# microsoft/GenerativeImage2Text

Hardware: AMD Instinct MI355X
Metric: captions/sec whole-node (GIT_BASE 224px bs=64/GPU greedy len=20) (higher is better)
Workload: dtype f16; 1 GPU; GIT_BASE 224px bs=64/GPU greedy max_len=20 frames=1; global_batch=64, parallelism=dp1, decode_steps_per_caption=19, seq_len_returned=20, hip_graph=True, contexts_in_flight=4, layernorm_folded=True, library=libgitmi_f16.so, encoder_chains=2, schedule=mixed

## Files before the change

generativeimage2text_amd/csrc/kernels_attn.hip:

```cpp
#include "gitmi_common.h"
#include "launchers.h"
#include <type_traits>

namespace gitmi {

constexpr int HD = 64;

template <typename T>
__global__ __launch_bounds__(256) void attn_full_valu_kernel(AttnFullArgs a) {
    __shared__ float Ks[64][HD + 1];
    __shared__ float Vs[64][HD + 1];
    __shared__ float qs[16][HD];
    __shared__ float ps[16][64];

    const int tid = threadIdx.x, lane = tid & 63, wave = tid >> 6;
    const int h = blockIdx.y, b = blockIdx.z;
    const int q0 = blockIdx.x * 16;
    const T* Q = reinterpret_cast<const T*>(a.q);
    const T* K = reinterpret_cast<const T*>(a.k);
    const T* V = reinterpret_cast<const T*>(a.v);
    T* O = reinterpret_cast<T*>(a.out);
    const size_t base_row = (size_t)b * a.N;
    const int n = a.ntok ? a.ntok[b] : a.N;
    if (q0 >= n) {
        for (int i = tid; i < 16 * HD; i += 256) {
            const int qr = q0 + i / HD;
            if (qr < a.N) st<T>(O + (base_row + qr) * a.ldo + h * HD + i % HD, 0.f);
        }
        return;
    }

    for (int i = tid; i < 16 * HD; i += 256) {
        const int qi = i / HD, d = i % HD;
        const int qr = q0 + qi;
        qs[qi][d] = qr < n ? ld<T>(Q + (base_row + qr) * a.ldq + h * HD + d) * a.scale : 0.f;
    }

    float m_run[4], l_run[4], o_acc[4];
#pragma unroll
    for (int j = 0; j < 4; ++j) { m_run[j] = -INFINITY; l_run[j] = 0.f; o_acc[j] = 0.f; }

    for (int kt = 0; kt < n; kt += 64) {
        __syncthreads();
        for (int i = tid; i < 64 * HD; i += 256) {
            const int key = i / HD, d = i % HD;
            const int kr = kt + key;
            float kv = 0.f, vv = 0.f;
            if (kr < n) {
                kv = ld<T>(K + (base_row + kr) * a.ldk + h * HD + d);
                vv = ld<T>(V + (base_row + kr) * a.ldv + h * HD + d);
            }
            Ks[key][d] = kv;
            Vs[key][d] = vv;
        }
        __syncthreads();
#pragma unroll
        for (int j = 0; j < 4; ++j) {
            const int qi = wave * 4 + j;
            float s = 0.f;
#pragma unroll 16
            for (int d = 0; d < HD; ++d) s += qs[qi][d] * Ks[lane][d];
            if (kt + lane >= n) s = -INFINITY;
            const float m_new = fmaxf(m_run[j], wave_max(s));
            const float p = __expf(s - m_new);
            const float alpha = __expf(m_run[j] - m_new);
            l_run[j] = l_run[j] * alpha + wave_sum(p);
            m_run[j] = m_new;
            ps[qi][lane] = p;
            __builtin_amdgcn_fence(__ATOMIC_RELEASE, "wavefront");
            __builtin_amdgcn_wave_barrier();
            __builtin_amdgcn_fence(__ATOMIC_ACQUIRE, "wavefront");
            float o = o_acc[j] * alpha;
#pragma unroll 16
            for (int key = 0; key < 64; ++key) o += ps[qi][key] * Vs[key][lane];
            o_acc[j] = o;
        }
    }
#pragma unroll
    for (int j = 0; j < 4; ++j) {
        const int qr = q0 + wave * 4 + j;
        if (qr < a.N) st<T>(O + (base_row + qr) * a.ldo + h * HD + lane, qr < n ? o_acc[j] / l_run[j] : 0.f);
    }
}

constexpr int FA_LDK = HD + 8;
constexpr int FA_LDV = 64 + 8;

__global__ __launch_bounds__(256) void attn_full_mfma_kernel(AttnFullArgs a) {
    __shared__ __attribute__((aligned(16))) bf16_t Ks[64 * FA_LDK];
    __shared__ __attribute__((aligned(16))) bf16_t Vt[HD * FA_LDV];

    constexpr int QT = 4;
    const int tid = threadIdx.x, lane = tid & 63, wave = tid >> 6;
    const int l15 = lane & 15, lg = lane >> 4;
    const int h = blockIdx.y, b = blockIdx.z;
    const int qbase = blockIdx.x * 256;
    const bf16_t* Q = reinterpret_cast<const bf16_t*>(a.q);
    const bf16_t* K = reinterpret_cast<const bf16_t*>(a.k);
    const bf16_t* V = reinterpret_cast<const bf16_t*>(a.v);
    bf16_t* O = reinterpret_cast<bf16_t*>(a.out);
    const size_t base_row = (size_t)b * a.N;
    const int n = a.ntok ? a.ntok[b] : a.N;

    bf16x8_t qf[QT][2];
    f32x4_t o_acc[QT][4];
    float m_run[QT], l_run[QT];
#pragma unroll
    for (int t = 0; t < QT; ++t) {
        int qr = qbase + (t * 4 + wave) * 16 + l15;
        qr = qr < n ? qr : n - 1;
        const bf16_t* qp = Q + (base_row + qr) * a.ldq + h * HD + lg * 8;
        qf[t][0] = *reinterpret_cast<const bf16x8_t*>(qp);
        qf[t][1] = *reinterpret_cast<const bf16x8_t*>(qp + 32);
#pragma unroll
        for (int dt = 0; dt < 4; ++dt) o_acc[t][dt] = f32x4_t{0.f, 0.f, 0.f, 0.f};
        m_run[t] = -INFINITY;
        l_run[t] = 0.f;
    }

    const int ld_row = tid >> 3;
    const int ld_c = (tid & 7) * 8;

    const int kend = qbase < n ? n : 0;
    for (int kt = 0; kt < kend; kt += 64) {
        __syncthreads();
#pragma unroll
        for (int it = 0; it < 2; ++it) {
            const int key = ld_row + it * 32;
            int kr = kt + key;
            kr = kr < n ? kr : n - 1;
            const u32x4_t kc = *reinterpret_cast<const u32x4_t*>(K + (base_row + kr) * a.ldk + h * HD + ld_c);
            const u32x4_t vc = *reinterpret_cast<const u32x4_t*>(V + (base_row + kr) * a.ldv + h * HD + ld_c);
            *reinterpret_cast<u32x4_t*>(Ks + key * FA_LDK + ld_c) = kc;
#pragma unroll
            for (int e = 0; e < 4; ++e) {
                Vt[(ld_c + 2 * e) * FA_LDV + key] = (bf16_t)(vc[e] & 0xffffu);
                Vt[(ld_c + 2 * e + 1) * FA_LDV + key] = (bf16_t)(vc[e] >> 16);
            }
        }
        __syncthreads();

#pragma unroll
        for (int t = 0; t < QT; ++t) {
            if (qbase + (t * 4 + wave) * 16 >= n) continue;
            f32x4_t s_acc[4];
#pragma unroll
            for (int st_ = 0; st_ < 4; ++st_) {
                s_acc[st_] = f32x4_t{0.f, 0.f, 0.f, 0.f};
#pragma unroll
                for (int ks = 0; ks < 2; ++ks) {
                    const bf16x8_t kf = *reinterpret_cast<const bf16x8_t*>(Ks + (st_ * 16 + l15) * FA_LDK + ks * 32 + lg * 8);
                    s_acc[st_] = mfma16(kf, qf[t][ks], s_acc[st_]);
                }
            }
            float tmax = -INFINITY;
#pragma unroll
            for (int st_ = 0; st_ < 4; ++st_)
#pragma unroll
                for (int r = 0; r < 4; ++r) {
                    const int key = kt + st_ * 16 + lg * 4 + r;
                    const float sv = key < n ? s_acc[st_][r] * a.scale : -INFINITY;
                    s_acc[st_][r] = sv;
                    tmax = fmaxf(tmax, sv);
                }
            tmax = fmaxf(tmax, __shfl_xor(tmax, 16, 64));
            tmax = fmaxf(tmax, __shfl_xor(tmax, 32, 64));
            const float m_new = fmaxf(m_run[t], tmax);
            const float alpha = fast_exp(m_run[t] - m_new);
            float psum = 0.f;
#pragma unroll
            for (int st_ = 0; st_ < 4; ++st_)
#pragma unroll
                for (int r = 0; r < 4; ++r) {
                    const float p = fast_exp(s_acc[st_][r] - m_new);
                    s_acc[st_][r] = p;
                    psum += p;
                }
            psum += __shfl_xor(psum, 16, 64);
            psum += __shfl_xor(psum, 32, 64);
            l_run[t] = l_run[t] * alpha + psum;
            m_run[t] = m_new;
#pragma unroll
            for (int dt = 0; dt < 4; ++dt)
#pragma unroll
                for (int r = 0; r < 4; ++r) o_acc[t][dt][r] *= alpha;

#pragma unroll
            for (int hf = 0; hf < 2; ++hf) {
                bf16x8_t pf;
                {
                    union { bf16x8_t v; uint32_t u[4]; } pk;
                    pk.u[0] = pack2bf(s_acc[2 * hf][0], s_acc[2 * hf][1]);
                    pk.u[1] = pack2bf(s_acc[2 * hf][2], s_acc[2 * hf][3]);
                    pk.u[2] = pack2bf(s_acc[2 * hf + 1][0], s_acc[2 * hf + 1][1]);
                    pk.u[3] = pack2bf(s_acc[2 * hf + 1][2], s_acc[2 * hf + 1][3]);
                    pf = pk.v;
                }
#pragma unroll
                for (int dt = 0; dt < 4; ++dt) {
                    union { bf16x8_t v; uint2 h2[2]; } vf;
                    const bf16_t* vp = Vt + (dt * 16 + l15) * FA_LDV + hf * 32 + lg * 4;
                    vf.h2[0] = *reinterpret_cast<const uint2*>(vp);
                    vf.h2[1] = *reinterpret_cast<const uint2*>(vp + 16);
                    o_acc[t][dt] = mfma16(vf.v, pf, o_acc[t][dt]);
                }
            }
        }
    }

#pragma unroll
    for (int t = 0; t < QT; ++t) {
        const int qr = qbase + (t * 4 + wave) * 16 + l15;
        if (qr < a.N) {
            const float inv = qr < n ? 1.0f / l_run[t] : 0.f;
            bf16_t* op = O + (base_row + qr) * a.ldo + h * HD;
#pragma unroll
            for (int dt = 0; dt < 4; ++dt) {
                uint2 tt;
                tt.x = pack2bf(o_acc[t][dt][0] * inv, o_acc[t][dt][1] * inv);
                tt.y = pack2bf(o_acc[t][dt][2] * inv, o_acc[t][dt][3] * inv);
                *reinterpret_cast<uint2*>(op + dt * 16 + lg * 4) = tt;
            }
        }
    }
}

template <int NSUB, bool RAGGED = false>
__global__ __launch_bounds__(256, 2) void attn_full_mfma_short_kernel(AttnFullArgs a) {
    constexpr int NK = NSUB * 16;
    constexpr int NB = (NSUB + 1) / 2;
    constexpr int LDV = NB * 32 + 8;
    static_assert((LDV / 8) % 2 == 1, "V^T row stride must be an odd multiple of 16 bytes");
    __shared__ __attribute__((aligned(16))) bf16_t Ks[NK * FA_LDK];
    __shared__ __attribute__((aligned(16))) bf16_t Vt[HD * LDV];

    const int tid = threadIdx.x, lane = tid & 63, wave = tid >> 6;
    const int l15 = lane & 15, lg = lane >> 4;
    const int h = blockIdx.x, b = blockIdx.y;
    const bf16_t* Q = reinterpret_cast<const bf16_t*>(a.q);
    const bf16_t* K = reinterpret_cast<const bf16_t*>(a.k);
    const bf16_t* V = reinterpret_cast<const bf16_t*>(a.v);
    bf16_t* O = reinterpret_cast<bf16_t*>(a.out);
    const size_t base_row = (size_t)b * a.N;
    const int n = RAGGED ? a.ntok[b] : a.N;
    if constexpr (RAGGED) {
        for (int i = tid; i < (a.N - n) * 8; i += 256) {
            const int qr = n + (i >> 3);
            *reinterpret_cast<u32x4_t*>(O + (base_row + qr) * a.ldo + h * HD + (i & 7) * 8) = u32x4_t{0u, 0u, 0u, 0u};
        }
    }

#pragma unroll
    for (int it = 0; it < (NK * 8 + 255) / 256; ++it) {
        int idx = tid + it * 256;
        const bool ok = idx < NK * 8;
        idx = ok ? idx : NK * 8 - 1;
        const int key = idx >> 3, c = idx & 7;
        const int kr = key < n ? key : n - 1;
        const u32x4_t kc = *reinterpret_cast<const u32x4_t*>(K + (base_row + kr) * a.ldk + h * HD + c * 8);
        if (ok) *reinterpret_cast<u32x4_t*>(Ks + key * FA_LDK + c * 8) = kc;
    }
#pragma unroll
    for (int it = 0; it < (NB * 8 * 8 + 255) / 256; ++it) {
        int task = tid + it * 256;
        const bool ok = task < NB * 8 * 8;
        task = ok ? task : NB * 8 * 8 - 1;
        const int kg = task % (NB * 8), c = task / (NB * 8);
        u32x4_t vc[4];
#pragma unroll
        for (int e = 0; e < 4; ++e) {
            const int key = kg * 4 + e;
            const int kr = key < n ? key : n - 1;
            vc[e] = *reinterpret_cast<const u32x4_t*>(V + (base_row + kr) * a.ldv + h * HD + c * 8);
            if (key >= n) vc[e] = u32x4_t{0u, 0u, 0u, 0u};
        }
        if (ok) {
#pragma unroll
            for (int w = 0; w < 4; ++w) {
                uint2 even, odd;
                even.x = (vc[0][w] & 0xffffu) | (vc[1][w] << 16);
                even.y = (vc[2][w] & 0xffffu) | (vc[3][w] << 16);
                odd.x = (vc[0][w] >> 16) | (vc[1][w] & 0xffff0000u);
                odd.y = (vc[2][w] >> 16) | (vc[3][w] & 0xffff0000u);
                *reinterpret_cast<uint2*>(Vt + (c * 8 + 2 * w) * LDV + kg * 4) = even;
                *reinterpret_cast<uint2*>(Vt + (c * 8 + 2 * w + 1) * LDV + kg * 4) = odd;
            }
        }
    }
    __syncthreads();

    const int nqt = (n + 15) >> 4;
    const float c2 = a.scale * 1.4426950408889634f;

    auto process = [&](auto nt_c, int t0) {
        constexpr int NT = decltype(nt_c)::value;
        bf16x8_t qf[NT][2];
#pragma unroll
        for (int u = 0; u < NT; ++u) {
            int qr = (t0 + 4 * u) * 16 + l15;
            qr = qr < n ? qr : n - 1;
            const bf16_t* qp = Q + (base_row + qr) * a.ldq + h * HD + lg * 8;
            qf[u][0] = *reinterpret_cast<const bf16x8_t*>(qp);
            qf[u][1] = *reinterpret_cast<const bf16x8_t*>(qp + 32);
        }
        f32x4_t sacc[NT][NSUB];
#pragma unroll
        for (int st_ = 0; st_ < NSUB; ++st_) {
            const bf16x8_t kf0 = *reinterpret_cast<const bf16x8_t*>(Ks + (st_ * 16 + l15) * FA_LDK + lg * 8);
            const bf16x8_t kf1 = *reinterpret_cast<const bf16x8_t*>(Ks + (st_ * 16 + l15) * FA_LDK + 32 + lg * 8);
#pragma unroll
            for (int u = 0; u < NT; ++u) {
                sacc[u][st_] = mfma16(kf0, qf[u][0], f32x4_t{0.f, 0.f, 0.f, 0.f});
                sacc[u][st_] = mfma16(kf1, qf[u][1], sacc[u][st_]);
            }
            if constexpr (NSUB > 13) { if (st_ % 4 == 3) __builtin_amdgcn_sched_barrier(0); }
        }
        float inv_l[NT];
#pragma unroll
        for (int u = 0; u < NT; ++u) {
            if constexpr (RAGGED) {
#pragma unroll
                for (int st_ = 0; st_ < NSUB; ++st_)
#pragma unroll
                    for (int r = 0; r < 4; ++r)
                        if (st_ * 16 + lg * 4 + r >= n) sacc[u][st_][r] = -INFINITY;
            } else {
#pragma unroll
                for (int r = 0; r < 4; ++r)
                    if ((NSUB - 1) * 16 + lg * 4 + r >= a.N) sacc[u][NSUB - 1][r] = -INFINITY;
            }
            float m = -INFINITY;
#pragma unroll
            for (int st_ = 0; st_ < NSUB; ++st_)
#pragma unroll
                for (int r = 0; r < 4; ++r) m = fmaxf(m, sacc[u][st_][r]);
            m = fmaxf(m, __shfl_xor(m, 16, 64));
            m = fmaxf(m, __shfl_xor(m, 32, 64));
            const float mc = m * c2;
            float psum = 0.f;
#pragma unroll
            for (int st_ = 0; st_ < NSUB; ++st_)
#pragma unroll
                for (int r = 0; r < 4; ++r) {
                    const float p = __builtin_amdgcn_exp2f(sacc[u][st_][r] * c2 - mc);
                    sacc[u][st_][r] = p;
                    psum += p;
                }
            psum += __shfl_xor(psum, 16, 64);
            psum += __shfl_xor(psum, 32, 64);
            inv_l[u] = 1.0f / psum;
        }
        uint32_t pk2[NT][NSUB][2];
#pragma unroll
        for (int u = 0; u < NT; ++u)
#pragma unroll
            for (int st_ = 0; st_ < NSUB; ++st_) {
                pk2[u][st_][0] = pack2bf(sacc[u][st_][0], sacc[u][st_][1]);
                pk2[u][st_][1] = pack2bf(sacc[u][st_][2], sacc[u][st_][3]);
            }
        f32x4_t o_acc[NT][4];
#pragma unroll
        for (int u = 0; u < NT; ++u)
#pragma unroll
            for (int dt = 0; dt < 4; ++dt) o_acc[u][dt] = f32x4_t{0.f, 0.f, 0.f, 0.f};
#pragma unroll
        for (int blk = 0; blk < NB; ++blk) {
            bf16x8_t pf[NT];
#pragma unroll
            for (int u = 0; u < NT; ++u) {
                union { bf16x8_t v; uint32_t w[4]; } pk;
                pk.w[0] = pk2[u][2 * blk][0];
                pk.w[1] = pk2[u][2 * blk][1];
                const bool has1 = 2 * blk + 1 < NSUB;
                const int s1 = has1 ? 2 * blk + 1 : 0;
                pk.w[2] = has1 ? pk2[u][s1][0] : 0u;
                pk.w[3] = has1 ? pk2[u][s1][1] : 0u;
                pf[u] = pk.v;
            }
#pragma unroll
            for (int dt = 0; dt < 4; ++dt) {
                union { bf16x8_t v; uint2 h2[2]; } vf;
                const bf16_t* vp = Vt + (dt * 16 + l15) * LDV + blk * 32 + lg * 4;
                vf.h2[0] = *reinterpret_cast<const uint2*>(vp);
                vf.h2[1] = *reinterpret_cast<const uint2*>(vp + 16);
#pragma unroll
                for (int u = 0; u < NT; ++u)
                    o_acc[u][dt] = mfma16(vf.v, pf[u], o_acc[u][dt]);
            }
        }
#pragma unroll
        for (int u = 0; u < NT; ++u) {
            const int qr = (t0 + 4 * u) * 16 + l15;
            if (qr < n) {
                bf16_t* op = O + (base_row + qr) * a.ldo + h * HD;
#pragma unroll
                for (int dt = 0; dt < 4; ++dt) {
                    uint2 tt;
                    tt.x = pack2bf(o_acc[u][dt][0] * inv_l[u], o_acc[u][dt][1] * inv_l[u]);
                    tt.y = pack2bf(o_acc[u][dt][2] * inv_l[u], o_acc[u][dt][3] * inv_l[u]);
                    *reinterpret_cast<uint2*>(op + dt * 16 + lg * 4) = tt;
                }
            }
        }
    };

    for (int t0 = wave; t0 < nqt; t0 += 8) {
        if (t0 + 4 < nqt) process(std::integral_constant<int, 2>{}, t0);
        else process(std::integral_constant<int, 1>{}, t0);
    }
}

template <typename T>
__global__ void kv_repack_kernel(const T* __restrict__ qkv, T* __restrict__ kh, T* __restrict__ vh, int B, int N, int H,
                                 int d) {
    constexpr int CH = 16 / (int)sizeof(T);
    constexpr int CPH = HD / CH;
    const size_t per = (size_t)B * H * N * CPH;
    for (size_t i = blockIdx.x * (size_t)blockDim.x + threadIdx.x; i < 2 * per; i += (size_t)gridDim.x * blockDim.x) {
        const int kv = i >= per;
        size_t r = kv ? i - per : i;
        const int c = (int)(r % CPH); r /= CPH;
        const int n = (int)(r % N); r /= N;
        const int h = (int)(r % H);
        const int b = (int)(r / H);
        const T* src = qkv + ((size_t)b * N + n) * 3 * d + (kv ? 2 : 1) * d + h * HD + c * CH;
        T* dst = (kv ? vh : kh) + (((size_t)b * H + h) * N + n) * HD + c * CH;
        *reinterpret_cast<u32x4_t*>(dst) = *reinterpret_cast<const u32x4_t*>(src);
    }
}

template <typename T> struct Raw8;
template <> struct Raw8<bf16_t> {
    u32x4_t r;
    __device__ __forceinline__ void load(const bf16_t* p) { r = *reinterpret_cast<const u32x4_t*>(p); }
    __device__ __forceinline__ void load_nt(const bf16_t* p) { r = __builtin_nontemporal_load(reinterpret_cast<const u32x4_t*>(p)); }
    __device__ __forceinline__ void store(bf16_t* p) const { *reinterpret_cast<u32x4_t*>(p) = r; }
    __device__ __forceinline__ void zero() { r = u32x4_t{0u, 0u, 0u, 0u}; }
    __device__ __forceinline__ void get(float (&v)[8]) const {
#pragma unroll
        for (int i = 0; i < 4; ++i) {
            unpack2op(r[i], v[2 * i], v[2 * i + 1]);
        }
    }
};
template <> struct Raw8<float> {
    f32x4_t a, b;
    __device__ __forceinline__ void load(const float* p) {
        a = *reinterpret_cast<const f32x4_t*>(p);
        b = *reinterpret_cast<const f32x4_t*>(p + 4);
    }
    __device__ __forceinline__ void load_nt(const float* p) {
        a = __builtin_nontemporal_load(reinterpret_cast<const f32x4_t*>(p));
        b = __builtin_nontemporal_load(reinterpret_cast<const f32x4_t*>(p + 4));
    }
    __device__ __forceinline__ void store(float* p) const {
        *reinterpret_cast<f32x4_t*>(p) = a;
        *reinterpret_cast<f32x4_t*>(p + 4) = b;
    }
    __device__ __forceinline__ void zero() { a = f32x4_t{0.f, 0.f, 0.f, 0.f}; b = a; }
    __device__ __forceinline__ void get(float (&v)[8]) const {
#pragma unroll
        for (int i = 0; i < 4; ++i) { v[i] = a[i]; v[4 + i] = b[i]; }
    }
};

template <typename T, int KB, int PF = 8, int TI = 5>
__global__ __launch_bounds__(256) void attn_decode_kernel(AttnDecodeArgs a) {
    __shared__ float part[4][KB][HD + 2];

    const int tid = threadIdx.x;
    const int h = blockIdx.x, b = blockIdx.y, H = gridDim.x;
    const int k = a.beams;
    const T* QKV = reinterpret_cast<const T*>(a.qkv);
    const T* IMGK = reinterpret_cast<const T*>(a.img_k);
    const T* IMGV = reinterpret_cast<const T*>(a.img_v);
    T* TK = reinterpret_cast<T*>(a.txt_k);
    T* TV = reinterpret_cast<T*>(a.txt_v);
    T* O = reinterpret_cast<T*>(a.out);
    const int ld3 = 3 * a.d;
    const int row0 = b * k;
    const int grp = tid >> 3, sub = tid & 7;
    const int wave = tid >> 6;

    const int bi = a.img_of ? a.img_of[b] : b;
    const int n_img = a.ntok ? a.ntok[bi] : a.N_img;
    const T* kbase = IMGK + ((size_t)bi * H + h) * a.N_img * HD + sub * 8;
    const T* vbase = IMGV + ((size_t)bi * H + h) * a.N_img * HD + sub * 8;
    const int nt = a.pos + 1;

    int t_j[TI], t_s[TI], t_row[TI];
#pragma unroll
    for (int u = 0; u < TI; ++u) {
        const int it = grp + 32 * u;
        t_j[u] = it < k * nt ? it / nt : -1;
        t_s[u] = it < k * nt ? it % nt : 0;
        if constexpr (KB == 1) t_row[u] = row0;
        else t_row[u] = (t_j[u] >= 0 && t_s[u] != a.pos) ? a.kv_src[(size_t)(row0 + t_j[u]) * a.ld_src + t_s[u]] : 0;
    }
    Raw8<T> qr[KB];
#pragma unroll
    for (int j = 0; j < KB; ++j) {
        if (j < k) qr[j].load(QKV + (size_t)(row0 + j) * ld3 + h * HD + sub * 8);
        else qr[j].zero();
    }
    Raw8<T> kr[PF], vr[PF];
#pragma unroll
    for (int u = 0; u < PF; ++u) {
        const int n = grp + 32 * u;
        if (n < n_img && !(a.dbg & 1)) { kr[u].load_nt(kbase + (size_t)n * HD); vr[u].load_nt(vbase + (size_t)n * HD); }
        else { kr[u].zero(); vr[u].zero(); }
    }
    Raw8<T> tk[TI], tv[TI];
#pragma unroll
    for (int u = 0; u < TI; ++u) {
        if (t_j[u] < 0) { tk[u].zero(); tv[u].zero(); }
        else if (t_s[u] == a.pos) {
            const T* src = QKV + (size_t)(row0 + t_j[u]) * ld3 + a.d + h * HD + sub * 8;
            tk[u].load(src);
            tv[u].load(src + a.d);
        } else {
            const size_t off = ((size_t)t_row[u] * a.T_max + t_s[u]) * a.d + h * HD + sub * 8;
            tk[u].load(TK + off);
            tv[u].load(TV + off);
        }
    }
    if (tid < k * 8) {
        const int j = tid >> 3;
        const T* src = QKV + (size_t)(row0 + j) * ld3 + a.d + h * HD + sub * 8;
        const size_t dst = ((size_t)(row0 + j) * a.T_max + a.pos) * a.d + h * HD + sub * 8;
        Raw8<T> ck, cv;
        ck.load(src);
        cv.load(src + a.d);
        ck.store(TK + dst);
        cv.store(TV + dst);
    }

    float q[KB][8], m[KB], l[KB], o[KB][8];
#pragma unroll
    for (int j = 0; j < KB; ++j) {
        qr[j].get(q[j]);
        m[j] = -INFINITY;
        l[j] = 0.f;
#pragma unroll
        for (int e = 0; e < 8; ++e) { q[j][e] *= a.scale; o[j][e] = 0.f; }
    }
    auto dot8 = [&](const float (&x)[8], const float (&y)[8]) {
        float p = 0.f;
#pragma unroll
        for (int e = 0; e < 8; ++e) p += x[e] * y[e];
        p += __shfl_xor(p, 1, 64);
        p += __shfl_xor(p, 2, 64);
        p += __shfl_xor(p, 4, 64);
        return p;
    };

    for (int base = 0; base < n_img; base += 32 * PF) {
        if (base > 0) {
#pragma unroll
            for (int u = 0; u < PF; ++u) {
                const int n = base + grp + 32 * u;
                if (n < n_img) { kr[u].load_nt(kbase + (size_t)n * HD); vr[u].load_nt(vbase + (size_t)n * HD); }
                else { kr[u].zero(); vr[u].zero(); }
            }
        }
        float sc[KB][PF];
        float cm[KB];
#pragma unroll
        for (int j = 0; j < KB; ++j) cm[j] = -INFINITY;
#pragma unroll
        for (int u = 0; u < PF; ++u) {
            const bool valid = base + grp + 32 * u < n_img;
            float kv[8];
            kr[u].get(kv);
#pragma unroll
            for (int j = 0; j < KB; ++j) {
                const float sv = valid ? dot8(q[j], kv) : -INFINITY;
                sc[j][u] = sv;
                cm[j] = fmaxf(cm[j], sv);
            }
        }
#pragma unroll
        for (int j = 0; j < KB; ++j) {
            if (cm[j] == -INFINITY) continue;
            const float mn = fmaxf(m[j], cm[j]);
            const float al = fast_exp(m[j] - mn);
            l[j] *= al;
#pragma unroll
            for (int e = 0; e < 8; ++e) o[j][e] *= al;
            m[j] = mn;
        }
#pragma unroll
        for (int u = 0; u < PF; ++u) {
            float vv[8];
            vr[u].get(vv);
#pragma unroll
            for (int j = 0; j < KB; ++j) {
                const float p = sc[j][u] == -INFINITY ? 0.f : fast_exp(sc[j][u] - m[j]);
                l[j] += p;
#pragma unroll
                for (int e = 0; e < 8; ++e) o[j][e] += p * vv[e];
            }
        }
    }
    auto text_item = [&](int jj, const float (&kv)[8], const float (&vv)[8]) {
#pragma unroll
        for (int j = 0; j < KB; ++j) {
            if (j == jj) {
                const float sv = dot8(q[j], kv);
                const float mn = fmaxf(m[j], sv);
                const float al = fast_exp(m[j] - mn);
                const float p = fast_exp(sv - mn);
                l[j] = l[j] * al + p;
#pragma unroll
                for (int e = 0; e < 8; ++e) o[j][e] = o[j][e] * al + p * vv[e];
                m[j] = mn;
            }
        }
    };
#pragma unroll
    for (int u = 0; u < TI; ++u) {
        if (t_j[u] >= 0) {
            float kv[8], vv[8];
            tk[u].get(kv);
            tv[u].get(vv);
            text_item(t_j[u], kv, vv);
        }
    }
    for (int it = grp + 32 * TI; it < k * nt; it += 32) {
        const int j = it / nt, sidx = it % nt;
        float kv[8], vv[8];
        if (sidx == a.pos) {
            ld8(QKV + (size_t)(row0 + j) * ld3 + a.d + h * HD + sub * 8, kv);
            ld8(QKV + (size_t)(row0 + j) * ld3 + 2 * a.d + h * HD + sub * 8, vv);
        } else {
            const int srow = KB == 1 ? row0 : a.kv_src[(size_t)(row0 + j) * a.ld_src + sidx];
            ld8(TK + ((size_t)srow * a.T_max + sidx) * a.d + h * HD + sub * 8, kv);
            ld8(TV + ((size_t)srow * a.T_max + sidx) * a.d + h * HD + sub * 8, vv);
        }
        text_item(j, kv, vv);
    }

#pragma unroll
    for (int j = 0; j < KB; ++j) {
#pragma unroll
        for (int off = 8; off < 64; off <<= 1) {
            const float m2 = __shfl_xor(m[j], off, 64);
            const float l2 = __shfl_xor(l[j], off, 64);
            const float mn = fmaxf(m[j], m2);
            const float a1 = m[j] == -INFINITY ? 0.f : fast_exp(m[j] - mn);
            const float a2 = m2 == -INFINITY ? 0.f : fast_exp(m2 - mn);
            l[j] = l[j] * a1 + l2 * a2;
#pragma unroll
            for (int e = 0; e < 8; ++e) {
                const float o2 = __shfl_xor(o[j][e], off, 64);
                o[j][e] = o[j][e] * a1 + o2 * a2;
            }
            m[j] = mn;
        }
        if ((tid & 63) < 8 && j < k) {
#pragma unroll
            for (int e = 0; e < 8; ++e) part[wave][j][sub * 8 + e] = o[j][e];
            if (sub == 0) { part[wave][j][HD] = m[j]; part[wave][j][HD + 1] = l[j]; }
        }
    }
    __syncthreads();
    for (int i = tid; i < k * HD; i += 256) {
        const int j = i / HD, dd = i % HD;
        float mm = -INFINITY;
#pragma unroll
        for (int w = 0; w < 4; ++w) mm = fmaxf(mm, part[w][j][HD]);
        float num = 0.f, den = 0.f;
#pragma unroll
        for (int w = 0; w < 4; ++w) {
            const float mw = part[w][j][HD];
            const float aw = mw == -INFINITY ? 0.f : fast_exp(mw - mm);
            num += aw * part[w][j][dd];
            den += aw * part[w][j][HD + 1];
        }
        if constexpr (sizeof(T) == 2) {
            if (a.out_frag) { O[frag_offset(row0 + j, h * HD + dd, a.d >> 5)] = f2bf(num / den); continue; }
        }
        st<T>(O + (size_t)(row0 + j) * a.d + h * HD + dd, num / den);
    }
}

hipError_t launch_attn_full(const AttnFullArgs& a, int B, bool is_f32, int impl, hipStream_t s) {
    if (B <= 0 || a.N <= 0) return hipSuccess;
    if (impl == 1) {
        if (is_f32) return hipErrorInvalidValue;
        const int nsub = (a.N + 15) / 16;
        if (nsub == 13 && a.ntok) hipLaunchKernelGGL((attn_full_mfma_short_kernel<13, true>), dim3(a.H, B), dim3(256), 0, s, a);
        else if (nsub == 13) hipLaunchKernelGGL(attn_full_mfma_short_kernel<13>, dim3(a.H, B), dim3(256), 0, s, a);
        else if (nsub == 17 && a.ntok) hipLaunchKernelGGL((attn_full_mfma_short_kernel<17, true>), dim3(a.H, B), dim3(256), 0, s, a);
        else if (nsub == 17) hipLaunchKernelGGL(attn_full_mfma_short_kernel<17>, dim3(a.H, B), dim3(256), 0, s, a);
        else hipLaunchKernelGGL(attn_full_mfma_kernel, dim3((a.N + 255) / 256, a.H, B), dim3(256), 0, s, a);
    } else if (impl == 2) {
        if (is_f32) return hipErrorInvalidValue;
        hipLaunchKernelGGL(attn_full_mfma_kernel, dim3((a.N + 255) / 256, a.H, B), dim3(256), 0, s, a);
    } else if (is_f32) {
        hipLaunchKernelGGL(attn_full_valu_kernel<float>, dim3((a.N + 15) / 16, a.H, B), dim3(256), 0, s, a);
    } else {
        hipLaunchKernelGGL(attn_full_valu_kernel<bf16_t>, dim3((a.N + 15) / 16, a.H, B), dim3(256), 0, s, a);
    }
    return hipGetLastError();
}

hipError_t launch_kv_repack(const void* qkv, void* kh, void* vh, int B, int N, int H, int d, hipStream_t s) {
    if (B <= 0 || N <= 0) return hipSuccess;
    const size_t total = 2 * (size_t)B * H * N * 16;
    size_t grid = (total + 255) / 256;
    grid = grid > 8192 ? 8192 : grid;
    hipLaunchKernelGGL(kv_repack_kernel<float>, dim3((int)grid), dim3(256), 0, s, (const float*)qkv, (float*)kh, (float*)vh, B, N,
                       H, d);
    return hipGetLastError();
}

hipError_t launch_attn_decode(const AttnDecodeArgs& a, int B, int H, hipStream_t s) {
    if (B <= 0) return hipSuccess;
    if (a.beams > 8) return hipErrorInvalidValue;
    if (a.beams <= 1) hipLaunchKernelGGL((attn_decode_kernel<float, 1>), dim3(H, B), dim3(256), 0, s, a);
    else if (a.beams <= 2) hipLaunchKernelGGL((attn_decode_kernel<float, 2>), dim3(H, B), dim3(256), 0, s, a);
    else if (a.beams <= 4) hipLaunchKernelGGL((attn_decode_kernel<float, 4>), dim3(H, B), dim3(256), 0, s, a);
    else hipLaunchKernelGGL((attn_decode_kernel<float, 8>), dim3(H, B), dim3(256), 0, s, a);
    return hipGetLastError();
}

}
```

Before: 11390 captions/s.

## Add persistent double-buffered walk kernel for short encoder attention

Adds a persistent attention kernel that gives each block several (head, batch) pairs. While one pair is being computed, the next pair's K/V is prefetched into a second LDS buffer with async global-to-LDS loads. V is read with LDS transpose loads on a swizzled layout, and Q loads are held across pairs. The existing short-kernel maths moves into a shared step function, and the new kernel becomes the default for non-ragged sequence lengths of 13 or 17 tiles. The cost is heavy LDS use, restricted occupancy and inline-asm wait counts that must be right for correctness. The last exp term uses a non-contracted multiply-subtract, apparently to keep numerics matching the old code.

```diff
diff --git a/generativeimage2text_amd/csrc/kernels_attn.hip b/generativeimage2text_amd/csrc/kernels_attn.hip
--- a/generativeimage2text_amd/csrc/kernels_attn.hip
+++ b/generativeimage2text_amd/csrc/kernels_attn.hip
@@ -225,6 +225,137 @@
     }
 }
 
+__device__ __forceinline__ float mul_then_sub(float a, float b, float c) {
+#pragma clang fp contract(off)
+    const float t = a * b;
+    return t - c;
+}
+
+template <int LDV>
+struct ShortVt {
+    const bf16_t* base;
+    struct Raw { bf16x8_t f[4]; };
+    __device__ __forceinline__ Raw load(int blk) const {
+        Raw r;
+#pragma unroll
+        for (int dt = 0; dt < 4; ++dt) {
+            union { bf16x8_t v; uint2 h2[2]; } vf;
+            const bf16_t* vp = base + dt * 16 * LDV + blk * 32;
+            vf.h2[0] = *reinterpret_cast<const uint2*>(vp);
+            vf.h2[1] = *reinterpret_cast<const uint2*>(vp + 16);
+            r.f[dt] = vf.v;
+        }
+        return r;
+    }
+    template <int PENDING> __device__ __forceinline__ void wait(Raw&) const {}
+    __device__ __forceinline__ bf16x8_t get(const Raw& r, int dt) const { return r.f[dt]; }
+};
+
+template <int NSUB, int NT, bool RAGGED, typename KF, typename VS>
+__device__ __forceinline__ void attn_short_step(const bf16x8_t (&qf)[NT][2], KF kfrag, const VS& vsrc, int nkeys, float c2, int lg,
+                                                uint2 (&outp)[NT][4]) {
+    constexpr int NB = (NSUB + 1) / 2;
+    f32x4_t sacc[NT][NSUB];
+#pragma unroll
+    for (int st_ = 0; st_ < NSUB; ++st_) {
+        const bf16x8_t kf0 = kfrag(st_, 0);
+        const bf16x8_t kf1 = kfrag(st_, 1);
+#pragma unroll
+        for (int u = 0; u < NT; ++u) {
+            sacc[u][st_] = mfma16(kf0, qf[u][0], f32x4_t{0.f, 0.f, 0.f, 0.f});
+            sacc[u][st_] = mfma16(kf1, qf[u][1], sacc[u][st_]);
+        }
+        if constexpr (NSUB > 13) { if (st_ % 4 == 3) __builtin_amdgcn_sched_barrier(0); }
+    }
+    float inv_l[NT];
+#pragma unroll
+    for (int u = 0; u < NT; ++u) {
+        if constexpr (RAGGED) {
+#pragma unroll
+            for (int st_ = 0; st_ < NSUB; ++st_)
+#pragma unroll
+                for (int r = 0; r < 4; ++r)
+                    if (st_ * 16 + lg * 4 + r >= nkeys) sacc[u][st_][r] = -INFINITY;
+        } else {
+#pragma unroll
+            for (int r = 0; r < 4; ++r)
+                if ((NSUB - 1) * 16 + lg * 4 + r >= nkeys) sacc[u][NSUB - 1][r] = -INFINITY;
+        }
+        float m = -INFINITY;
+#pragma unroll
+        for (int st_ = 0; st_ < NSUB; ++st_)
+#pragma unroll
+            for (int r = 0; r < 4; ++r) m = fmaxf(m, sacc[u][st_][r]);
+        m = fmaxf(m, __shfl_xor(m, 16, 64));
+        m = fmaxf(m, __shfl_xor(m, 32, 64));
+        const float mc = m * c2;
+        float psum = 0.f;
+#pragma unroll
+        for (int st_ = 0; st_ < NSUB; ++st_)
+#pragma unroll
+            for (int r = 0; r < 4; ++r) {
+                const bool last = st_ == NSUB - 1 && r == 3;
+                const float p = __builtin_amdgcn_exp2f(last ? mul_then_sub(sacc[u][st_][r], c2, mc)
+                                                            : __builtin_fmaf(sacc[u][st_][r], c2, -mc));
+                sacc[u][st_][r] = p;
+                psum += p;
+            }
+        psum += __shfl_xor(psum, 16, 64);
+        psum += __shfl_xor(psum, 32, 64);
+        inv_l[u] = 1.0f / psum;
+    }
+    uint32_t pk2[NT][NSUB][2];
+#pragma unroll
+    for (int u = 0; u < NT; ++u)
+#pragma unroll
+        for (int st_ = 0; st_ < NSUB; ++st_) {
+            pk2[u][st_][0] = pack2bf(sacc[u][st_][0], sacc[u][st_][1]);
+            pk2[u][st_][1] = pack2bf(sacc[u][st_][2], sacc[u][st_][3]);
+        }
+    f32x4_t o_acc[NT][4];
+#pragma unroll
+    for (int u = 0; u < NT; ++u)
+#pragma unroll
+        for (int dt = 0; dt < 4; ++dt) o_acc[u][dt] = f32x4_t{0.f, 0.f, 0.f, 0.f};
+    typename VS::Raw vraw[2];
+    vraw[0] = vsrc.load(0);
+#pragma unroll
+    for (int blk = 0; blk < NB; ++blk) {
+        if (blk + 1 < NB) {
+            vraw[(blk + 1) & 1] = vsrc.load(blk + 1);
+            vsrc.template wait<8>(vraw[blk & 1]);
+        } else {
+            vsrc.template wait<0>(vraw[blk & 1]);
+        }
+        bf16x8_t pf[NT];
+#pragma unroll
+        for (int u = 0; u < NT; ++u) {
+            union { bf16x8_t v; uint32_t w[4]; } pk;
+            pk.w[0] = pk2[u][2 * blk][0];
+            pk.w[1] = pk2[u][2 * blk][1];
+            const bool has1 = 2 * blk + 1 < NSUB;
+            const int s1 = has1 ? 2 * blk + 1 : 0;
+            pk.w[2] = has1 ? pk2[u][s1][0] : 0u;
+            pk.w[3] = has1 ? pk2[u][s1][1] : 0u;
+            pf[u] = pk.v;
+        }
+#pragma unroll
+        for (int dt = 0; dt < 4; ++dt) {
+            const bf16x8_t vf = vsrc.get(vraw[blk & 1], dt);
+#pragma unroll
+            for (int u = 0; u < NT; ++u)
+                o_acc[u][dt] = mfma16(vf, pf[u], o_acc[u][dt]);
+        }
+    }
+#pragma unroll
+    for (int u = 0; u < NT; ++u)
+#pragma unroll
+        for (int dt = 0; dt < 4; ++dt) {
+            outp[u][dt].x = pack2bf(o_acc[u][dt][0] * inv_l[u], o_acc[u][dt][1] * inv_l[u]);
+            outp[u][dt].y = pack2bf(o_acc[u][dt][2] * inv_l[u], o_acc[u][dt][3] * inv_l[u]);
+        }
+}
+
 template <int NSUB, bool RAGGED = false>
 __global__ __launch_bounds__(256, 2) void attn_full_mfma_short_kernel(AttnFullArgs a) {
     constexpr int NK = NSUB * 16;
@@ -303,103 +434,20 @@
             qf[u][0] = *reinterpret_cast<const bf16x8_t*>(qp);
             qf[u][1] = *reinterpret_cast<const bf16x8_t*>(qp + 32);
         }
-        f32x4_t sacc[NT][NSUB];
-#pragma unroll
-        for (int st_ = 0; st_ < NSUB; ++st_) {
-            const bf16x8_t kf0 = *reinterpret_cast<const bf16x8_t*>(Ks + (st_ * 16 + l15) * FA_LDK + lg * 8);
-            const bf16x8_t kf1 = *reinterpret_cast<const bf16x8_t*>(Ks + (st_ * 16 + l15) * FA_LDK + 32 + lg * 8);
-#pragma unroll
-            for (int u = 0; u < NT; ++u) {
-                sacc[u][st_] = mfma16(kf0, qf[u][0], f32x4_t{0.f, 0.f, 0.f, 0.f});
-                sacc[u][st_] = mfma16(kf1, qf[u][1], sacc[u][st_]);
-            }
-            if constexpr (NSUB > 13) { if (st_ % 4 == 3) __builtin_amdgcn_sched_barrier(0); }
-        }
-        float inv_l[NT];
-#pragma unroll
-        for (int u = 0; u < NT; ++u) {
-            if constexpr (RAGGED) {
-#pragma unroll
-                for (int st_ = 0; st_ < NSUB; ++st_)
-#pragma unroll
-                    for (int r = 0; r < 4; ++r)
-                        if (st_ * 16 + lg * 4 + r >= n) sacc[u][st_][r] = -INFINITY;
-            } else {
-#pragma unroll
-                for (int r = 0; r < 4; ++r)
-                    if ((NSUB - 1) * 16 + lg * 4 + r >= a.N) sacc[u][NSUB - 1][r] = -INFINITY;
-            }
-            float m = -INFINITY;
-#pragma unroll
-            for (int st_ = 0; st_ < NSUB; ++st_)
-#pragma unroll
-                for (int r = 0; r < 4; ++r) m = fmaxf(m, sacc[u][st_][r]);
-            m = fmaxf(m, __shfl_xor(m, 16, 64));
-            m = fmaxf(m, __shfl_xor(m, 32, 64));
-            const float mc = m * c2;
-            float psum = 0.f;
-#pragma unroll
-            for (int st_ = 0; st_ < NSUB; ++st_)
-#pragma unroll
-                for (int r = 0; r < 4; ++r) {
-                    const float p = __builtin_amdgcn_exp2f(sacc[u][st_][r] * c2 - mc);
-                    sacc[u][st_][r] = p;
-                    psum += p;
-                }
-            psum += __shfl_xor(psum, 16, 64);
-            psum += __shfl_xor(psum, 32, 64);
-            inv_l[u] = 1.0f / psum;
-        }
-        uint32_t pk2[NT][NSUB][2];
-#pragma unroll
-        for (int u = 0; u < NT; ++u)
-#pragma unroll
-            for (int st_ = 0; st_ < NSUB; ++st_) {
-                pk2[u][st_][0] = pack2bf(sacc[u][st_][0], sacc[u][st_][1]);
-                pk2[u][st_][1] = pack2bf(sacc[u][st_][2], sacc[u][st_][3]);
-            }
-        f32x4_t o_acc[NT][4];
-#pragma unroll
-        for (int u = 0; u < NT; ++u)
-#pragma unroll
-            for (int dt = 0; dt < 4; ++dt) o_acc[u][dt] = f32x4_t{0.f, 0.f, 0.f, 0.f};
-#pragma unroll
-        for (int blk = 0; blk < NB; ++blk) {
-            bf16x8_t pf[NT];
-#pragma unroll
-            for (int u = 0; u < NT; ++u) {
-                union { bf16x8_t v; uint32_t w[4]; } pk;
-                pk.w[0] = pk2[u][2 * blk][0];
-                pk.w[1] = pk2[u][2 * blk][1];
-                const bool has1 = 2 * blk + 1 < NSUB;
-                const int s1 = has1 ? 2 * blk + 1 : 0;
-                pk.w[2] = has1 ? pk2[u][s1][0] : 0u;
-                pk.w[3] = has1 ? pk2[u][s1][1] : 0u;
-                pf[u] = pk.v;
-            }
-#pragma unroll
-            for (int dt = 0; dt < 4; ++dt) {
-                union { bf16x8_t v; uint2 h2[2]; } vf;
-                const bf16_t* vp = Vt + (dt * 16 + l15) * LDV + blk * 32 + lg * 4;
-                vf.h2[0] = *reinterpret_cast<const uint2*>(vp);
-                vf.h2[1] = *reinterpret_cast<const uint2*>(vp + 16);
-#pragma unroll
-                for (int u = 0; u < NT; ++u)
-                    o_acc[u][dt] = mfma16(vf.v, pf[u], o_acc[u][dt]);
-            }
-        }
+        uint2 outp[NT][4];
+        attn_short_step<NSUB, NT, RAGGED>(
+            qf,
+            [&](int st_, int half) {
+                return *reinterpret_cast<const bf16x8_t*>(Ks + (st_ * 16 + l15) * FA_LDK + half * 32 + lg * 8);
+            },
+            ShortVt<LDV>{Vt + l15 * LDV + lg * 4}, RAGGED ? n : a.N, c2, lg, outp);
 #pragma unroll
         for (int u = 0; u < NT; ++u) {
             const int qr = (t0 + 4 * u) * 16 + l15;
             if (qr < n) {
                 bf16_t* op = O + (base_row + qr) * a.ldo + h * HD;
 #pragma unroll
-                for (int dt = 0; dt < 4; ++dt) {
-                    uint2 tt;
-                    tt.x = pack2bf(o_acc[u][dt][0] * inv_l[u], o_acc[u][dt][1] * inv_l[u]);
-                    tt.y = pack2bf(o_acc[u][dt][2] * inv_l[u], o_acc[u][dt][3] * inv_l[u]);
-                    *reinterpret_cast<uint2*>(op + dt * 16 + lg * 4) = tt;
-                }
+                for (int dt = 0; dt < 4; ++dt) *reinterpret_cast<uint2*>(op + dt * 16 + lg * 4) = outp[u][dt];
             }
         }
     };
@@ -408,6 +456,168 @@
         if (t0 + 4 < nqt) process(std::integral_constant<int, 2>{}, t0);
         else process(std::integral_constant<int, 1>{}, t0);
     }
+}
+
+constexpr int WK_WAVES = 8;
+typedef __attribute__((address_space(3))) void walk_lds_void_t;
+typedef __attribute__((ext_vector_type(4))) short walk_s16x4_t;
+__device__ __forceinline__ int walk_swz(int row) { return ((row >> 1) & 3) << 1; }
+__device__ __forceinline__ void walk_lds_barrier() {
+    asm volatile("s_waitcnt lgkmcnt(0)" ::: "memory");
+    __builtin_amdgcn_s_barrier();
+    asm volatile("" ::: "memory");
+}
+
+struct WalkV {
+    uint32_t addr;
+    struct Raw { walk_s16x4_t h[4][2]; };
+    __device__ __forceinline__ Raw load(int blk) const {
+        Raw r;
+#pragma unroll
+        for (int dt = 0; dt < 4; ++dt) {
+            const uint32_t p = (addr ^ (uint32_t)(dt << 5)) + (uint32_t)blk * 4096u;
+            asm volatile("ds_read_b64_tr_b16 %0, %1" : "=v"(r.h[dt][0]) : "v"(p));
+            asm volatile("ds_read_b64_tr_b16 %0, %1 offset:2048" : "=v"(r.h[dt][1]) : "v"(p));
+        }
+        return r;
+    }
+    template <int PENDING> __device__ __forceinline__ void wait(Raw& r) const {
+        asm volatile("s_waitcnt lgkmcnt(%8)"
+                     : "+v"(r.h[0][0]), "+v"(r.h[0][1]), "+v"(r.h[1][0]), "+v"(r.h[1][1]), "+v"(r.h[2][0]), "+v"(r.h[2][1]),
+                       "+v"(r.h[3][0]), "+v"(r.h[3][1])
+                     : "n"(PENDING));
+    }
+    __device__ __forceinline__ bf16x8_t get(const Raw& r, int dt) const {
+        union { bf16x8_t v; walk_s16x4_t h4[2]; } vf;
+        vf.h4[0] = r.h[dt][0];
+        vf.h4[1] = r.h[dt][1];
+        return vf.v;
+    }
+};
+
+template <int NSUB>
+__global__ __launch_bounds__(64 * WK_WAVES) void attn_full_walk_kernel(AttnFullArgs a, int n_pairs) {
+    constexpr int NK = NSUB * 16;
+    constexpr int NB = (NSUB + 1) / 2;
+    constexpr int NV = NB * 32;
+    constexpr int KBYTES = NK * 128, BUF = (NK + NV) * 128;
+    constexpr int PK = NK / 8, PV = NV / 8;
+    static_assert(2 * BUF <= 160 * 1024, "two buffers must fit the CU's LDS");
+    __shared__ __attribute__((aligned(1024))) unsigned char smem[2 * BUF];
+
+    const int tid = threadIdx.x, lane = tid & 63;
+    const int wave = __builtin_amdgcn_readfirstlane(tid >> 6);
+    const int l15 = lane & 15, lg = lane >> 4;
+    const bf16_t* Q = reinterpret_cast<const bf16_t*>(a.q);
+    const bf16_t* K = reinterpret_cast<const bf16_t*>(a.k);
+    const bf16_t* V = reinterpret_cast<const bf16_t*>(a.v);
+    bf16_t* O = reinterpret_cast<bf16_t*>(a.out);
+    const int N = a.N;
+    const int G = (int)gridDim.x, w = (int)blockIdx.x;
+    const int npw = w < n_pairs ? (n_pairs - 1 - w) / G + 1 : 0;
+    const int pvn = (N + 7) >> 3;
+    const float c2 = a.scale * 1.4426950408889634f;
+
+    const int r8 = lane >> 3;
+    const int src_c = ((lane & 7) ^ walk_swz(r8)) * 8;
+    auto issue_pair = [&](int ord) {
+        const int pair = w + ord * G;
+        const int h = pair % a.H, b = pair / a.H;
+        const size_t base_row = (size_t)b * N;
+        unsigned char* buf = smem + (ord & 1) * BUF;
+        for (int j = wave; j < PK + pvn; j += WK_WAVES) {
+            const bool isv = j >= PK;
+            const int piece = isv ? j - PK : j;
+            int row = piece * 8 + r8;
+            row = row < N ? row : N - 1;
+            const bf16_t* src = (isv ? V + (base_row + row) * a.ldv : K + (base_row + row) * a.ldk) + h * HD + src_c;
+            __builtin_amdgcn_global_load_lds((const void*)src, (walk_lds_void_t*)(buf + (isv ? KBYTES : 0) + piece * 1024), 16, 0, 0);
+        }
+    };
+    auto load_q = [&](int ord, int t0, auto& qf) {
+        const int pair = w + ord * G;
+        const int h = pair % a.H, b = pair / a.H;
+#pragma unroll
+        for (int u = 0; u < (int)(sizeof(qf) / sizeof(qf[0])); ++u) {
+            int qr = (t0 + WK_WAVES * u) * 16 + l15;
+            qr = qr < N ? qr : N - 1;
+            const bf16_t* qp = Q + ((size_t)b * N + qr) * a.ldq + h * HD + lg * 8;
+            qf[u][0] = *reinterpret_cast<const bf16x8_t*>(qp);
+            qf[u][1] = *reinterpret_cast<const bf16x8_t*>(qp + 32);
+        }
+    };
+    auto store_out = [&](int ord, int t0, const auto& outp) {
+        const int pair = w + ord * G;
+        const int h = pair % a.H, b = pair / a.H;
+#pragma unroll
+        for (int u = 0; u < (int)(sizeof(outp) / sizeof(outp[0])); ++u) {
+            const int qr = (t0 + WK_WAVES * u) * 16 + l15;
+            if (qr < N) {
+                bf16_t* op = O + ((size_t)b * N + qr) * a.ldo + h * HD;
+#pragma unroll
+                for (int dt = 0; dt < 4; ++dt) *reinterpret_cast<uint2*>(op + dt * 16 + lg * 4) = outp[u][dt];
+            }
+        }
+    };
+
+    if (npw == 0) return;
+    issue_pair(0);
+    for (int i = tid; i < 2 * (PV - pvn) * 64; i += 64 * WK_WAVES) {
+        const int bsel = i >= (PV - pvn) * 64, o = i - bsel * (PV - pvn) * 64;
+        *reinterpret_cast<u32x4_t*>(smem + bsel * BUF + KBYTES + pvn * 1024 + o * 16) = u32x4_t{0u, 0u, 0u, 0u};
+    }
+
+    const int k_off = l15 * 128 + ((lg ^ walk_swz(l15)) << 4);
+    const int vq = l15 >> 2, vp = l15 & 3;
+    const int v_row = lg * 4 + vq;
+    const int v_off = KBYTES + v_row * 128 + ((((vp >> 1) ^ walk_swz(v_row)) << 4) | ((vp & 1) << 3));
+
+    auto walk = [&](auto nt_c) {
+        constexpr int NT = decltype(nt_c)::value;
+        constexpr bool HOLD = NSUB <= 13;
+        bf16x8_t qn[NT][2];
+        uint2 outp[NT][4];
+        if constexpr (HOLD) load_q(0, wave, qn);
+        for (int ord = 0; ord < npw; ++ord) {
+            unsigned char* buf = smem + (ord & 1) * BUF;
+            asm volatile("s_waitcnt vmcnt(0)" ::: "memory");
+            if ((N & 7) && wave == (PK + (N >> 3)) % WK_WAVES && r8 >= (N & 7))
+                *reinterpret_cast<u32x4_t*>(buf + KBYTES + (N >> 3) * 1024 + lane * 16) = u32x4_t{0u, 0u, 0u, 0u};
+            walk_lds_barrier();
+            if constexpr (!HOLD) load_q(ord, wave, qn);
+            bf16x8_t qf[NT][2];
+#pragma unroll
+            for (int u = 0; u < NT; ++u) {
+                qf[u][0] = qn[u][0]; qf[u][1] = qn[u][1];
+                asm volatile("" : "+v"(qf[u][0]), "+v"(qf[u][1]) : : "memory");
+            }
+            if (HOLD && ord > 0) store_out(ord - 1, wave, outp);
+            if (ord + 1 < npw) {
+                issue_pair(ord + 1);
+                if constexpr (HOLD) load_q(ord + 1, wave, qn);
+            }
+            asm volatile("" ::: "memory");
+            auto kfrag = [&](int st_, int half) {
+                return *reinterpret_cast<const bf16x8_t*>(buf + ((k_off ^ (half << 6)) + st_ * 2048));
+            };
+            const WalkV vsrc{(uint32_t)(size_t)(__attribute__((address_space(3))) unsigned char*)buf + (uint32_t)v_off};
+            attn_short_step<NSUB, NT, false>(qf, kfrag, vsrc, N, c2, lg, outp);
+            if constexpr (!HOLD) store_out(ord, wave, outp);
+            if constexpr (NSUB > 2 * WK_WAVES) {
+                static_assert(NSUB <= 2 * WK_WAVES + 1, "one extra tile at most");
+                if (wave == 0) {
+                    bf16x8_t q1[1][2];
+                    uint2 o1[1][4];
+                    load_q(ord, 2 * WK_WAVES, q1);
+                    attn_short_step<NSUB, 1, false>(q1, kfrag, vsrc, N, c2, lg, o1);
+                    store_out(ord, 2 * WK_WAVES, o1);
+                }
+            }
+        }
+        if constexpr (HOLD) store_out(npw - 1, wave, outp);
+    };
+    if (wave + WK_WAVES < NSUB) walk(std::integral_constant<int, 2>{});
+    else walk(std::integral_constant<int, 1>{});
 }
 
 template <typename T>
@@ -686,10 +896,18 @@
 
 hipError_t launch_attn_full(const AttnFullArgs& a, int B, bool is_f32, int impl, hipStream_t s) {
     if (B <= 0 || a.N <= 0) return hipSuccess;
-    if (impl == 1) {
+    const int walk_grid = impl >> 8;
+    impl &= 255;
+    if (impl == 1 || impl == 3) {
         if (is_f32) return hipErrorInvalidValue;
         const int nsub = (a.N + 15) / 16;
-        if (nsub == 13 && a.ntok) hipLaunchKernelGGL((attn_full_mfma_short_kernel<13, true>), dim3(a.H, B), dim3(256), 0, s, a);
+        if (impl == 1 && !a.ntok && (nsub == 13 || nsub == 17)) {
+            const int pairs = a.H * B;
+            const int grid = walk_grid > 0 ? (walk_grid < pairs ? walk_grid : pairs) : (pairs < 256 ? pairs : 256);
+            if (nsub == 13) hipLaunchKernelGGL(attn_full_walk_kernel<13>, dim3(grid), dim3(64 * WK_WAVES), 0, s, a, pairs);
+            else hipLaunchKernelGGL(attn_full_walk_kernel<17>, dim3(grid), dim3(64 * WK_WAVES), 0, s, a, pairs);
+        }
+        else if (nsub == 13 && a.ntok) hipLaunchKernelGGL((attn_full_mfma_short_kernel<13, true>), dim3(a.H, B), dim3(256), 0, s, a);
         else if (nsub == 13) hipLaunchKernelGGL(attn_full_mfma_short_kernel<13>, dim3(a.H, B), dim3(256), 0, s, a);
         else if (nsub == 17 && a.ntok) hipLaunchKernelGGL((attn_full_mfma_short_kernel<17, true>), dim3(a.H, B), dim3(256), 0, s, a);
         else if (nsub == 17) hipLaunchKernelGGL(attn_full_mfma_short_kernel<17>, dim3(a.H, B), dim3(256), 0, s, a);
```

New measurement: 11440 captions/s (median of 3 runs). No clear change (+0.4%).
